# michaelnny/alpha_zero

Measured on AMD Instinct MI355X. Metric: self-play moves/sec (whole node), 9x9 Go @ 200 sims/move, higher is better.
Workload: dtype fp32-class evaluator (f16 hi+lo pairs, 3 MFMA products, fp32 accumulate) / f32-f64 tree

## Files before the change

alpha_zero_amd/csrc/azsp_hip.hip:

```cpp
#include <hip/hip_runtime.h>
#include <stdlib.h>

#include <type_traits>

#include "azsp_impl.h"
#include "az_conv64.h"
#include "az_conv19.h"
#include "az_conv_sp.h"
#include "az_conv_sp17.h"
#include "az_resblock_sp17.h"
#include "az_conv_sp2p.h"
#include "az_conv_spg.h"

static hipError_t g_last = hipSuccess;
#define AZ_HIP(x) ((g_last = (x)) == hipSuccess ? 0 : -1)

template <int N, int GAME, class Op>
__global__ void __launch_bounds__(256) k_game(const AzCfg c, const AzMem m, const Op op, const int g0, const int g1) {
    __shared__ typename Engine<WaveDev, N, GAME>::SC sc[4];
    const int wave = (int)(threadIdx.x >> 6);
    const int g = g0 + (int)blockIdx.x * 4 + wave;
    if (g >= g1) return;
    Engine<WaveDev, N, GAME> e(c, m, g, sc[wave]);
    op(e);
}

__global__ void __launch_bounds__(256) k_dihedral(const DihedralArgs a, long long total) {
    for (long long t = (long long)blockIdx.x * blockDim.x + threadIdx.x; t < total; t += (long long)gridDim.x * blockDim.x)
        az_dihedral_elem(a, t);
}

__global__ void __launch_bounds__(256) k_replay_gather(const ReplayGatherArgs a, long long total) {
    for (long long t = (long long)blockIdx.x * blockDim.x + threadIdx.x; t < total; t += (long long)gridDim.x * blockDim.x)
        az_replay_gather_elem(a, t);
}

__global__ void __launch_bounds__(256) k_bias_act(const BiasActArgs a) {
    for (long long i = (long long)blockIdx.x * blockDim.x + threadIdx.x; i < a.nvec; i += (long long)gridDim.x * blockDim.x)
        az_bias_act_vec(a, i);
}

__global__ void __launch_bounds__(1024) k_harvest_scan(const int* __restrict__ len, int* __restrict__ ofs, int* __restrict__ counts, int n2, int rot,
                                                        int cap, int max_games) {
    __shared__ int ss[1024], sg[1024], best[2];
    const int t = (int)threadIdx.x, per = (n2 + 1023) / 1024, lo = t * per < n2 ? t * per : n2, hi = lo + per < n2 ? lo + per : n2;
    int s = 0, g = 0;
    for (int i = lo; i < hi; ++i) {
        const int l = len[(i + rot) % n2];
        s += l;
        g += l > 0;
    }
    ss[t] = s;
    sg[t] = g;
    if (t < 2) best[t] = 0;
    __syncthreads();
    for (int d = 1; d < 1024; d <<= 1) {
        const int a = t >= d ? ss[t - d] : 0, b = t >= d ? sg[t - d] : 0;
        __syncthreads();
        ss[t] += a;
        sg[t] += b;
        __syncthreads();
    }
    int mine[2] = {0, 0};
    az_harvest_scan_range(len, ofs, n2, rot, cap, max_games, lo, hi, ss[t] - s, sg[t] - g, mine);
    if (mine[1] > 0) {
        atomicMax(&best[0], mine[0]);
        atomicMax(&best[1], mine[1]);
    }
    __syncthreads();
    if (t < 2) counts[t] = best[t];
}

namespace azb {
void* alloc(size_t n) {
    void* p = nullptr;
    if (AZ_HIP(hipMalloc(&p, n))) return nullptr;
    if (AZ_HIP(hipMemset(p, 0, n))) {
        hipFree(p);
        return nullptr;
    }
    return p;
}
void release(void* p) { (void)hipFree(p); }
int h2d(void* d, const void* s, size_t n, void* st) {
    if (AZ_HIP(hipMemcpyAsync(d, s, n, hipMemcpyHostToDevice, (hipStream_t)st))) return -1;
    return AZ_HIP(hipStreamSynchronize((hipStream_t)st));
}
int d2h(void* d, const void* s, size_t n, void* st) {
    if (AZ_HIP(hipMemcpyAsync(d, s, n, hipMemcpyDeviceToHost, (hipStream_t)st))) return -1;
    return AZ_HIP(hipStreamSynchronize((hipStream_t)st));
}
int zero(void* d, size_t n, void* st) { return AZ_HIP(hipMemsetAsync(d, 0, n, (hipStream_t)st)); }
int sync(void* st) { return AZ_HIP(hipStreamSynchronize((hipStream_t)st)); }
void* host_alloc(size_t n) {
    void* p = nullptr;
    return AZ_HIP(hipHostMalloc(&p, n, hipHostMallocDefault)) ? nullptr : p;
}
void host_release(void* p) { (void)hipHostFree(p); }
int set_device(int dev) {
    int n = 0;
    if (AZ_HIP(hipGetDeviceCount(&n)) || n < 1) return -1;
    return AZ_HIP(hipSetDevice(dev));
}
const char* backend_error() { return hipGetErrorString(g_last); }
template <class K, class... A> static int launch_k(K* kernel, unsigned grid, unsigned block, size_t lds, void* st, const A&... args) {
    hipLaunchKernelGGL(kernel, dim3(grid), dim3(block), lds, (hipStream_t)st, args...);
    return AZ_HIP(hipGetLastError());
}
template <class F> static int with_flag(bool flag, F&& f) { return flag ? f(std::true_type{}) : f(std::false_type{}); }
template <class F> static int with_flag(bool f0, bool f1, F&& f) {
    return with_flag(f0, [&](auto F0) { return with_flag(f1, [&](auto F1) { return f(decltype(F0){}, F1); }); });
}
static int cu_count() {
    static int n_cu = 0;
    if (n_cu == 0) {
        int dev = 0;
        hipDeviceProp_t prop;
        if (hipGetDevice(&dev) != hipSuccess || hipGetDeviceProperties(&prop, dev) != hipSuccess) return -1;
        n_cu = prop.multiProcessorCount > 0 ? prop.multiProcessorCount : 256;
    }
    return n_cu;
}
static int persistent_grid(long long units, int k = 1) {
    const int n_cu = cu_count();
    if (n_cu < 0) return -1;
    const long long slots = n_cu / k > 0 ? n_cu / k : 1;
    return k * (int)(units < slots ? units : slots);
}
template <int N, int GAME, class Op> int launch(const AzCfg& c, const AzMem& m, const Op& op, void* st, int g0, int g1) {
    return launch_k(k_game<N, GAME, Op>, (unsigned)((g1 - g0 + 3) / 4), 256, 0, st, c, m, op, g0, g1);
}
int launch_dihedral(const DihedralArgs& a, long long total, void* st) {
    long long blocks = (total + 255) / 256;
    if (blocks > 2048) blocks = 2048;
    return launch_k(k_dihedral, (unsigned)blocks, 256, 0, st, a, total);
}
int launch_replay_gather(const ReplayGatherArgs& a, long long total, void* st) {
    long long blocks = (total + 255) / 256;
    if (blocks > 256 * 16) blocks = 256 * 16;
    return launch_k(k_replay_gather, (unsigned)blocks, 256, 0, st, a, total);
}
int launch_harvest_scan(const int* len, int* ofs, int* counts, int n2, int rot, int cap, int max_games, void* st) {
    return launch_k(k_harvest_scan, 1, 1024, 0, st, len, ofs, counts, n2, rot, cap, max_games);
}
int launch_bias_act(const BiasActArgs& a, void* st) {
    long long blocks = (a.nvec + 255) / 256;
    if (blocks > 256 * 32) blocks = 256 * 32;
    return launch_k(k_bias_act, (unsigned)blocks, 256, 0, st, a);
}
int launch_conv3x3_tiled(const void* x, const void* w, const float* bias, const void* res, void* y, long long boards, int S, int C,
                         int relu, void* st, int f16) {
    if (f16 && (S != CV_S || C != CV_C)) return 1;
    const auto xb = (const unsigned char*)x, rb = (const unsigned char*)res;
    const auto wb = (const unsigned short*)w;
    const auto yb = (unsigned char*)y;
    if (C == C6_C && (S == 17 || S == 9)) {
        const long long ntiles = S == 17 ? boards : (boards + 2) / 3;
        const int grid = persistent_grid(ntiles);
        if (grid < 0) return -1;
        return with_flag(S == 17, res != nullptr, [&](auto G17, auto RES) {
            return launch_k(k_conv3x3_t64<C6Geo<G17 ? 17 : 9>, RES, 8>, grid, CW_THREADS, 0, st, xb, wb, bias, rb, yb, (int)ntiles, relu);
        });
    }
    if (S == C9_S && C == 256) {
        static const bool two_launch = getenv("AZSP_CONV19_TWO_LAUNCH") != nullptr;
        const int grid = persistent_grid(boards, two_launch ? 4 : 8);
        if (grid < 0) return -1;
        if (x == y || res == y) return 1;
        if (!two_launch) {
            return with_flag(res != nullptr, [&](auto RES) {
                return launch_k(k_conv3x3_op19q<RES>, grid, CW_THREADS, 0, st, xb, wb, bias, rb, yb, (int)boards, relu);
            });
        }
        const int rc = with_flag(res != nullptr, [&](auto RES) {
            return launch_k(k_conv3x3_hb19<RES, 16>, grid, CW_THREADS, 0, st, xb, wb, bias, rb, yb, (int)boards, 0, 1, 256, 0, 32, 0);
        });
        if (rc) return rc;
        return launch_k(k_conv3x3_hb19<true, 16>, grid, CW_THREADS, 0, st, xb, wb, bias, (const unsigned char*)yb, yb, (int)boards, relu, 0, 256, 128, 32, 16);
    }
    if (S != CV_S || C != CV_C) return 1;
    const long long ntiles = (boards + CV_TB - 1) / CV_TB;
    const int grid = persistent_grid(ntiles);
    if (grid < 0) return -1;
    return with_flag(res != nullptr, f16 != 0, [&](auto RES, auto F16) {
        return launch_k(k_conv3x3_tiled<RES, 16, F16>, grid, CW_THREADS, 0, st, xb, wb, bias, rb, yb, (int)ntiles, relu);
    });
}
int launch_resblock_tiled(const void* x, const void* w1, const float* b1, const void* w2, const float* b2, void* y, long long boards, int S, int C,
                          void* st) {
    if (C != C6_C || (S != 17 && S != 9)) return 1;
    const long long ntiles = S == 17 ? boards : (boards + 2) / 3;
    const int grid = persistent_grid(ntiles);
    if (grid < 0) return -1;
    return with_flag(S == 17, [&](auto G17) {
        return launch_k(k_resblock64<C6Geo<G17 ? 17 : 9>>, grid, CW_THREADS, 0, st, (const unsigned char*)x, (const unsigned short*)w1, b1,
                        (const unsigned short*)w2, b2, (unsigned char*)y, (int)ntiles);
    });
}
int launch_stem_tiled(const void* x, const void* w, const float* bias, void* y, long long boards, int S, int C, int pad, int relu, void* st, int f16) {
    if (f16 && (S != CV_S || C != CV_C || pad != 1)) return 1;
    const bool t64 = C == C6_C && ((S == 13 && pad == 3) || (S == 9 && pad == 1)), go19 = S == C9_S && C == 256 && pad == 1;
    if (!t64 && !go19 && (S != CV_S || C != CV_C || pad != 1)) return 1;
    const long long ntiles = t64 ? (S == 13 ? boards : (boards + 2) / 3) : go19 ? boards : (boards + CV_TB - 1) / CV_TB;
    const int grid = persistent_grid(ntiles, go19 ? 4 : 1);
    if (grid < 0) return -1;
    const auto xb = (const unsigned char*)x, nores = (const unsigned char*)nullptr;
    const auto wb = (const unsigned short*)w;
    const auto yb = (unsigned char*)y;
    if (t64)
        return with_flag(S == 13, [&](auto G17) {
            return launch_k(k_conv3x3_t64<C6Geo<G17 ? 17 : 9>, false, 4>, grid, CW_THREADS, 0, st, xb, wb, bias, nores, yb, (int)ntiles, relu);
        });
    if (go19) return launch_k(k_conv3x3_hb19<false, 4>, grid, CW_THREADS, 0, st, xb, wb, bias, nores, yb, (int)boards, relu, 1, 32, 0, 4, 0);
    return with_flag(f16 != 0, [&](auto F16) {
        return launch_k(k_conv3x3_tiled<false, 4, F16>, grid, CW_THREADS, 0, st, xb, wb, bias, nores, yb, (int)ntiles, relu);
    });
}
int launch_head_tiled(const void* x, const float* w, const float* bias, void* pol, void* val, long long boards, int S, int C, int npol, int nval,
                      int pol_stride, int val_stride, void* st, int f16) {
    if (C % 8 || C > 1024 || npol + nval != 3) return 1;
    const long long npos = boards * S * S;
    return with_flag(f16 != 0, [&](auto F16) {
        return launch_k(k_head_tiled<3, F16>, (unsigned)((npos + 255) / 256), 256, 0, st, (const unsigned char*)x, w, bias, (unsigned short*)pol,
                        (unsigned short*)val, npos, npol, C, S * S, cv_tile_boards(S) * S * S, pol_stride, val_stride);
    });
}
template <int T1, int T2, bool F16> static int launch_fc_heads_t(const FcHeadsArgs& a, void* st) {
    return launch_k(k_fc_heads<T1, T2, F16>, (unsigned)((a.boards + 127) / 128), 256, 0, st, (const unsigned short*)a.pol, (const unsigned short*)a.val,
                    (const unsigned short*)a.wp, a.bp, a.ks1, (const unsigned short*)a.w1, a.b1, a.ks2, a.w2, a.b2, a.priors, a.values, a.boards, a.A);
}
int launch_fc_heads(const FcHeadsArgs& a, void* st) {
    const int nt1 = (a.A + 31) / 32, nt2 = (a.F + 31) / 32;
    if (a.f16) return nt1 == 3 && nt2 == 4 ? launch_fc_heads_t<3, 4, true>(a, st) : 1;
    if (nt1 == 3 && nt2 == 2) return launch_fc_heads_t<3, 2, false>(a, st);
    if (nt1 == 3 && nt2 == 4) return launch_fc_heads_t<3, 4, false>(a, st);
    if (nt1 == 6 && nt2 == 2) return launch_fc_heads_t<6, 2, false>(a, st);
    if (nt1 == 6 && nt2 == 4) return launch_fc_heads_t<6, 4, false>(a, st);
    if (nt1 == 12 && nt2 == 8) return launch_fc_heads_t<12, 8, false>(a, st);
    return 1;
}
int launch_tile_layout(const void* src, void* dst, long long boards, int S, int C, int to_tiled, void* st) {
    if (C % 8 || S < 1) return 1;
    const int nch = C / 8, tile_rows = cv_tile_boards(S) * S * S;
    const long long nchunks = boards * S * S * nch;
    return launch_k(k_tile_layout, (unsigned)((nchunks + 255) / 256), 256, 0, st, (const unsigned char*)src, (unsigned char*)dst, nchunks, to_tiled, nch,
                    tile_rows);
}
int launch_split_layout(const void* src, void* dst, long long boards, int S, int C, int to_split, void* st, unsigned* range) {
    if (C % 8 || S < 1) return 1;
    const long long nchunks = boards * S * S * (C / 8);
    return launch_k(k_split_layout, (unsigned)((nchunks + 255) / 256), 256, 0, st, (const unsigned char*)src, (unsigned char*)dst, nchunks, to_split, C / 8,
                    S * S, range);
}
template <bool RES, int NCH, int NCG, bool XLO0 = false>
static int launch_sp(const void* x, const void* w, const float* bias, const void* res, void* y, long long boards, int relu, void* st, unsigned* range) {
    const int grid = persistent_grid(boards, NCG);
    if (grid < 0) return -1;
    return launch_k(k_conv3x3_sp<RES, NCH, NCG, XLO0>, grid, CW_THREADS, 0, st, (const unsigned char*)x, (const _Float16*)w, bias, (const unsigned char*)res,
                    (unsigned char*)y, (int)boards, relu, range);
}
template <bool RES, int NCH, bool XLO0 = false>
static int launch_sp17(const void* x, const void* w, const float* bias, const void* res, void* y, long long boards, int relu, void* st, unsigned* range) {
    const int grid = persistent_grid(boards);
    if (grid < 0) return -1;
    return launch_k(k_conv3x3_sp17<RES, NCH, XLO0>, grid, CW_THREADS, 0, st, (const unsigned char*)x, (const _Float16*)w, bias, (const unsigned char*)res,
                    (unsigned char*)y, (int)boards, relu, range);
}
static long long spg_wave_items(long long boards, int S, int C, int NT, int NJ) {
    const long long nct = ((long long)S * S + 15) / 16;
    return boards * ((nct + NJ - 1) / NJ) * (C / (16 * NT));
}
static unsigned spg_wave_grid(long long boards, int S, int C, int NT, int NJ) {
    const long long grid = (spg_wave_items(boards, S, C, NT, NJ) + 3) / 4;
    return grid > 0x7fffffffLL ? 0u : (unsigned)grid;
}
template <bool RES, int KSUB, int NT, int NJ, int HALVES>
static int launch_spg_t(const void* x, const void* w, const float* bias, const void* res, void* y, long long boards, int S, int C, int relu, void* st,
                        unsigned* range) {
    const unsigned grid = spg_wave_grid(boards, S, C, NT, NJ);
    if (!grid) return 1;
    return launch_k(k_conv3x3_spg<RES, KSUB, NT, NJ, HALVES>, grid, 256, 0, st, (const unsigned char*)x, (const _Float16*)w, bias,
                    (const unsigned char*)(RES ? res : nullptr), (unsigned char*)y, (int)boards, S, C, relu, range);
}
template <bool RES, int KSUB, int NT>
static int launch_spgw_t(const void* x, const void* w, const float* bias, const void* res, void* y, long long boards, int S, int C, int relu, void* st,
                         unsigned* range) {
    const long long nct = ((long long)S * S + 15) / 16, grid = (boards * ((nct + 2) / 3) * (C / (64 * NT)) + 7) / 8 * 8;
    if (grid > 0x7fffffffLL || C % (64 * NT)) return 1;
    return launch_k(k_conv3x3_spgw<RES, KSUB, NT>, (unsigned)grid, 256, 0, st, (const unsigned char*)x, (const _Float16*)w, bias,
                    (const unsigned char*)(RES ? res : nullptr), (unsigned char*)y, (int)boards, S, C, relu, range);
}
template <int KSUB, int HALVES>
static int launch_spg_k(const void* x, const void* w, const float* bias, const void* res, void* y, long long boards, int S, int C, int relu, void* st,
                        unsigned* range, bool latency) {
    constexpr int NT = KSUB == 2 ? 1 : 2;
    return with_flag(res != nullptr, [&](auto RES) {
        return latency || HALVES == 2 ? launch_spg_t<RES, KSUB, 1, 2, HALVES>(x, w, bias, res, y, boards, S, C, relu, st, range)
                                      : launch_spgw_t<RES, KSUB, NT>(x, w, bias, res, y, boards, S, C, relu, st, range);
    });
}
static int launch_spg(const void* x, const void* w, const float* bias, const void* res, void* y, long long boards, int S, int C, int relu, void* st,
                      unsigned* range, bool latency, int halves) {
    if (S < 3 || S > 64 || boards < 1 || boards > 0x7fffffffLL) return 1;
    if (C == 64) return launch_spg_k<2, 1>(x, w, bias, res, y, boards, S, C, relu, st, range, latency);
    if (C == 128)
        return halves == 2 ? launch_spg_k<4, 2>(x, w, bias, res, y, boards, S, C, relu, st, range, latency)
                           : launch_spg_k<4, 1>(x, w, bias, res, y, boards, S, C, relu, st, range, latency);
    if (C == 256) return launch_spg_k<8, 1>(x, w, bias, res, y, boards, S, C, relu, st, range, latency);
    return 1;
}
static constexpr long long SPG_DEFAULT_WAVES = 1024;
static long long& spg_max_waves() {
    static long long n = [] {
        const char* e = getenv("AZSP_SPG_MAX_WAVES");
        const long long v = e ? atoll(e) : SPG_DEFAULT_WAVES;
        return v < 0 ? 0LL : v;
    }();
    return n;
}
static bool small_batch(long long boards, int S, int C) { return spg_wave_items(boards, S, C, 1, 2) <= spg_max_waves(); }
long long small_batch_waves(long long n) {
    const long long old = spg_max_waves();
    if (n >= 0) spg_max_waves() = n;
    return old;
}
int launch_conv3x3_split(const void* x, const void* w, const float* bias, const void* res, void* y, long long boards, int S, int C, int relu,
                         void* st, unsigned* range) {
    const bool sp17 = S == Sp17Geo::S && C == 64, sp9 = S == SpGeo9::S && (C == 128 || C == 64), small = small_batch(boards, S, C);
    if (!(sp17 || sp9) || small) return launch_spg(x, w, bias, res, y, boards, S, C, relu, st, range, small, sp9 && C == 128 ? 2 : 1);
    if (sp17)
        return with_flag(res != nullptr, [&](auto RES) { return launch_sp17<RES, 8>(x, w, bias, res, y, boards, relu, st, range); });
    if (C == 64) return with_flag(res != nullptr, [&](auto RES) { return launch_sp<RES, 8, 1>(x, w, bias, res, y, boards, relu, st, range); });
    const long long pairs = boards / 2;
    const int pgrid = persistent_grid(pairs, 2);
    if (pgrid < 0) return -1;
    const size_t off = (size_t)(2 * pairs) * 2 * 128 * SpGeo9::P2 * 2;
    const auto xb = (const unsigned char*)x, rb = (const unsigned char*)res;
    const auto yb = (unsigned char*)y;
    const int rc = with_flag(res != nullptr, [&](auto RES) {
        return pairs > 0 ? launch_k(k_conv3x3_sp2p<RES>, pgrid, CW_THREADS, 0, st, xb, (const _Float16*)w, bias, rb, yb, (int)pairs, relu, range) : 0;
    });
    if (rc || !(boards & 1)) return rc;
    return launch_spg(xb + off, w, bias, res ? rb + off : nullptr, yb + off, 1, S, C, relu, st, range, true, 2);
}
enum Scratch {
    SCRATCH_SPG_BLOCK,
    SCRATCH_COUNT
};
static constexpr long long SPG_SCRATCH_BOARDS = 256;
static void* device_scratch(Scratch which, size_t bytes) {
    static void* buf[SCRATCH_COUNT][16] = {};
    int dev = 0;
    if (hipGetDevice(&dev) != hipSuccess || dev < 0 || dev >= 16) return nullptr;
    if (!buf[which][dev] && AZ_HIP(hipMalloc(&buf[which][dev], bytes))) return nullptr;
    return buf[which][dev];
}
static int launch_resblock_spg(const unsigned char* x, const void* w1, const float* b1, const void* w2, const float* b2, unsigned char* y, long long boards,
                               int S, int C, void* st, unsigned* range) {
    void* mid = device_scratch(SCRATCH_SPG_BLOCK, (size_t)SPG_SCRATCH_BOARDS * 2 * 8 * Sb17::S * Sb17::S * 16);
    if (!mid) return -1;
    const int rc = launch_spg(x, w1, b1, nullptr, mid, boards, S, C, 1, st, range, true, 1);
    if (rc) return rc;
    return launch_spg(mid, w2, b2, x, y, boards, S, C, 1, st, range, true, 1);
}
int launch_resblock_split(const void* x, const void* w1, const float* b1, const void* w2, const float* b2, void* y, long long boards, int S, int C,
                          void* st, unsigned* range) {
    if (C != 64 || (S != Sb17::S && S != Sb9::S)) return 1;
    const long long pairs = boards / 2;
    const int grid = persistent_grid(S == Sb9::S ? pairs : boards);
    if (grid < 0) return -1;
    const auto xb = (const unsigned char*)x;
    const auto yb = (unsigned char*)y;
    if (small_batch(boards, S, C) && boards <= SPG_SCRATCH_BOARDS) return launch_resblock_spg(xb, w1, b1, w2, b2, yb, boards, S, C, st, range);
    if (S == Sb17::S) return launch_k(k_resblock_sp<Sb17, 6>, grid, CW_THREADS, 0, st, xb, (const _Float16*)w1, b1, (const _Float16*)w2, b2, yb, (int)boards, range);
    if (pairs > 0 && launch_k(k_resblock_sp<Sb9, 6>, grid, CW_THREADS, 0, st, xb, (const _Float16*)w1, b1, (const _Float16*)w2, b2, yb, (int)pairs, range)) return -1;
    if (!(boards & 1)) return 0;
    const size_t off = (size_t)(boards - 1) * Sb9::GTILEB;
    return launch_resblock_spg(xb + off, w1, b1, w2, b2, yb + off, 1, S, C, st, range);
}
int launch_split_features(const float* src, void* dst, long long boards, int S, int cin, void* st, unsigned* range) {
    if (cin < 1 || cin > 32 || S < 1) return 1;
    const long long nitems = boards * 4 * S * S;
    return launch_k(k_split_features, (unsigned)((nitems + 255) / 256), 256, 0, st, src, (unsigned char*)dst, nitems, cin, S * S, range);
}
template <bool XLO0>
static int launch_stem_spg(const void* x, const void* w, const float* bias, void* y, long long boards, int n, int C, int pad, int relu, void* st,
                           unsigned* range) {
    constexpr int NT = 1, NJ = 2;
    const int off = pad - 1, S = n + 2 * off;
    if ((pad != 1 && pad != 3) || n < 1 || S < 3 || S > 64 || (C != 64 && C != 128 && C != 256) || boards < 1 || boards > 0x7fffffffLL) return 1;
    const unsigned grid = spg_wave_grid(boards, S, C, NT, NJ);
    if (!grid) return 1;
    return launch_k(k_stem_spg<XLO0, NT, NJ>, grid, 256, 0, st, (const unsigned char*)x, (const _Float16*)w, bias, (unsigned char*)y, (int)boards, n, off,
                    C, relu, range);
}
static constexpr bool STEM_SPG_DEFAULT_SMALL = false;
int launch_stem_split(const void* x, const void* w, const float* bias, void* y, long long boards, int S, int C, int pad, int relu, void* st,
                      int x_lo_zero, unsigned* range) {
    const bool sp17 = S == 13 && C == 64 && pad == 3;
    const bool sp9 = S == SpGeo9::S && (C == 128 || C == 64) && pad == 1;
    const bool small = (pad == 1 || pad == 3) && small_batch(boards, S + 2 * (pad - 1), C) && (STEM_SPG_DEFAULT_SMALL || spg_max_waves() > SPG_DEFAULT_WAVES);
    return with_flag(x_lo_zero != 0, [&](auto XLO0) {
        if (!(sp17 || sp9) || small) return launch_stem_spg<XLO0>(x, w, bias, y, boards, S, C, pad, relu, st, range);
        if (sp17) return launch_sp17<false, 4, XLO0>(x, w, bias, nullptr, y, boards, relu, st, range);
        return C == 128 ? launch_sp<false, 4, 2, XLO0>(x, w, bias, nullptr, y, boards, relu, st, range)
                        : launch_sp<false, 4, 1, XLO0>(x, w, bias, nullptr, y, boards, relu, st, range);
    });
}
int split_range_read(const unsigned* rec, unsigned out[2], int reset, void* st) {
    void* p = (void*)rec;
    if (!p && AZ_HIP(hipGetSymbolAddress(&p, HIP_SYMBOL(g_sp_range)))) return -1;
    if (AZ_HIP(hipMemcpyAsync(out, p, 2 * sizeof(unsigned), hipMemcpyDeviceToHost, (hipStream_t)st))) return -1;
    if (reset && AZ_HIP(hipMemsetAsync(p, 0, 2 * sizeof(unsigned), (hipStream_t)st))) return -1;
    return AZ_HIP(hipStreamSynchronize((hipStream_t)st));
}
template <int BPB> static int launch_head_split_bpb(const HeadSplitArgs& a, void* st) {
    const int P2 = a.S * a.S;
    const size_t lds = (size_t)(BPB * (3 * ((P2 + 3) & ~3) + a.A + a.F)) * sizeof(float);
    if (lds > 64 * 1024) return 1;
    return launch_k(k_head_split<BPB>, (unsigned)((a.boards + BPB - 1) / BPB), 256, lds, st, (const unsigned char*)a.x, a.hw, a.hb, a.wp_t, a.bp, a.w1_t, a.b1, a.w2,
                    a.b2, a.priors, a.values, a.boards, a.C, P2, a.A, a.F, a.npol);
}
int launch_head_split(const HeadSplitArgs& a, void* st) {
    if (a.C % 8 || a.npol < 1 || a.npol > 2) return 1;
    return launch_head_split_bpb<4>(a, st);
}
}
```

Baseline: 7347.

## Add dedicated persistent pipelined stem conv kernel for 9x9 boards with 128 channels

Adds a specialized persistent stem kernel for 9x9, 128-channel, 32-input-channel boards. It keeps weights resident in registers, streams boards through an LDS ring with asynchronous DMA, and interleaves each board's epilogue stores with the next board's MFMA products. Corner cells are gathered into a side buffer and computed in batches of 16 boards. The goal is to hide load and store latency that the generic sp stem path exposes, at the cost of a lot of hand-scheduled code, high register pressure and one block per CU.

```diff
diff --git a/alpha_zero_amd/csrc/az_stem_sp9.h b/alpha_zero_amd/csrc/az_stem_sp9.h
--- /dev/null
+++ b/alpha_zero_amd/csrc/az_stem_sp9.h
@@ -0,0 +1,273 @@
+#pragma once
+#include <type_traits>
+
+#include "az_conv_sp.h"
+
+#if defined(__HIPCC__)
+#ifndef SP9_RING
+#define SP9_RING 4
+#endif
+#ifndef SP9_CELL16
+#define SP9_CELL16 true
+#endif
+
+template <bool XLO0> struct Sp9K {
+    typedef SpGeo9 G;
+    static constexpr int NR = SP9_RING;
+    static constexpr int NCH = 4, C = 128, CIN = 32, KS = 9, R = 3, NT = G::NCT;
+    static constexpr int NPROD = XLO0 ? 2 : 3, NQ = 2 * NPROD;
+    static constexpr int NPL = XLO0 ? 1 : 2;
+    static constexpr int LBLK = G::CELLS * 16, LPLANE = NCH * LBLK, LBUF = NPL * LPLANE;
+    static constexpr int GBLK = G::P2 * 16, XPLANE = NCH * GBLK, XTILE = 2 * XPLANE;
+    static constexpr int YPLANE = (C / 8) * GBLK, YTILE = 2 * YPLANE;
+    static constexpr int NP = (G::CELLS + 63) / 64, SPW = NPL * NCH / 4, NPW = NP * SPW;
+    static constexpr int NST = SP9_CELL16 ? 2 : 4;
+    static constexpr int ARITH = 2 * 2 * sp_epi_pair(false), CT_OPS = ARITH + NST;
+    static constexpr int S0 = 6;
+    static constexpr int BAR_T = KS - (R - 1);
+    typedef SpSpread<CT_OPS, S0, KS * NQ - 4 - S0> SpreadMid;
+    typedef SpSpread<CT_OPS, S0, BAR_T * NQ - S0> SpreadLast;
+    static constexpr int SIDE_BOARD = 8 * NCH * 16 + 16, SIDE0 = NR * LBUF + 16, LDS_BYTES = SIDE0 + 16 * SIDE_BOARD;
+    static constexpr int VM_PIECES = (NR - 2) * NPW, VM_COUNT = VM_PIECES + NT * NST * (NR - 2) + (NT - 1) * NST, VM_STEADY = VM_COUNT < 62 ? VM_COUNT : 62;
+    static_assert(NR >= 2 && NR <= 8, "ring depth");
+    static_assert((NT * KS) % R == 0, "a board's k-steps keep the fragment ring's phase");
+    static_assert(LPLANE + (2 * G::PITCH + 2) * 16 < 65536, "fragment addresses are a base + a 16-bit immediate");
+    static_assert(LDS_BYTES <= 160 * 1024, "LDS budget");
+};
+
+template <bool XLO0> __global__ void __launch_bounds__(CW_THREADS, 1)
+k_stem_sp9(const unsigned char* __restrict__ x, const _Float16* __restrict__ w, const float* __restrict__ bias, unsigned char* __restrict__ y,
+           int ntiles, int relu, unsigned* range) {
+    typedef SpGeo9 G;
+    typedef Sp9K<XLO0> K;
+    constexpr int NR = K::NR, NCH = K::NCH, C = K::C, CIN = K::CIN, KS = K::KS, R = K::R, NT = K::NT, NPROD = K::NPROD, NQ = K::NQ, NPL = K::NPL;
+    constexpr int LBLK = K::LBLK, LPLANE = K::LPLANE, LBUF = K::LBUF, GBLK = K::GBLK, XTILE = K::XTILE, YPLANE = K::YPLANE, YTILE = K::YTILE;
+    constexpr int NP = K::NP, SPW = K::SPW, NPW = K::NPW, NST = K::NST, ARITH = K::ARITH, CT_OPS = K::CT_OPS;
+    constexpr int SIDE_BOARD = K::SIDE_BOARD, SIDE0 = K::SIDE0;
+    constexpr int NF = 2 * KS * 2;
+    __shared__ __attribute__((aligned(1024))) unsigned char lds[K::LDS_BYTES];
+    const int tid = threadIdx.x, lane = tid & 63, l15 = lane & 15, kg = lane >> 4;
+    const int wave = __builtin_amdgcn_readfirstlane(tid >> 6);
+    const unsigned lds0 = (unsigned)(size_t)(__attribute__((address_space(3))) unsigned char*)lds;
+    const int slot = (int)blockIdx.x, nslot = (int)gridDim.x;
+    for (int i = tid; i < K::LDS_BYTES / 16; i += CW_THREADS) *(cv_u32x4*)(lds + i * 16) = (cv_u32x4){0u, 0u, 0u, 0u};
+    CV_BARRIER();
+    if (slot >= ntiles) return;
+
+    sp_f16x8 wf[NF];
+#pragma unroll
+    for (int f = 0; f < NF; ++f) {
+        const int r = f & 1, pt = f >> 1;
+        wf[f] = *(const sp_f16x8*)(w + ((size_t)(pt * C + wave * 32 + 8 * (l15 >> 2) + (l15 & 3) + 4 * r)) * CIN + kg * 8);
+    }
+    c6_f32x4 bv[2];
+#pragma unroll
+    for (int r = 0; r < 2; ++r)
+#pragma unroll
+        for (int e = 0; e < 4; ++e) bv[r][e] = bias[wave * 32 + 8 * kg + 4 * r + e];
+    const float lo_relu = relu ? 0.0f : -__builtin_inff();
+    const float lo_clamp = relu ? 0.0f : -SP_F16_MAX;
+
+    unsigned dsrc[NP];
+    unsigned long long dmask[NP];
+    sp_dma_plan(dsrc, dmask, lane, [](int cell) { return cell < G::CELLS ? G::pos_of_cell(cell) * 16 : -1; });
+    auto dma_board = [&](long long tile, int rs) __attribute__((always_inline)) {
+        const bool live = tile < ntiles;
+        const unsigned char* src = x + (size_t)(live ? tile : slot) * XTILE;
+        const unsigned dst = lds0 + (unsigned)(rs * LBUF);
+#pragma unroll
+        for (int i = 0; i < NPW; ++i) sp_dma_piece(src, dst, SPW * wave + i / NP, i % NP, GBLK, LBLK, live ? dmask[i % NP] : 0ull, dsrc[i % NP]);
+    };
+    unsigned lmap[NT], omap[NT];
+#pragma unroll
+    for (int j = 0; j < NT; ++j) {
+        const int pos = sp_map9.pos[j * 16 + l15];
+        lmap[j] = (unsigned)((G::PITCH * (pos / G::S) + pos % G::S) * 16 + kg * LBLK);
+        omap[j] = (unsigned)(pos * 16 + kg * GBLK);
+    }
+    auto out_off = [&](int j) __attribute__((always_inline)) {
+        unsigned v = omap[j];
+        asm volatile("" : "+v"(v));
+        return v;
+    };
+    sp_f16x8 bb[R][2];
+    auto load_frag = [&](unsigned img, int j, int t, int rs, int pl) __attribute__((always_inline)) {
+        bb[rs][pl] = *(const sp_f16x8*)(lds + img + lmap[j] + sp_frag_off(t, 1, G::PITCH, LBLK) + pl * LPLANE);
+    };
+
+#pragma unroll
+    for (int b = 0; b < NR; ++b) dma_board(slot + (long long)b * nslot, b);
+    asm volatile("s_waitcnt vmcnt(%0)" ::"n"((NR - 1) * NPW) : "memory");
+    CV_BARRIER();
+#pragma unroll
+    for (int s = 0; s < R - 1; ++s)
+#pragma unroll
+        for (int pl = 0; pl < NPL; ++pl) load_frag(0u, 0, s, s, pl);
+#pragma unroll
+    for (int f = 0; f < NF; ++f) asm volatile("" : : "a"(wf[f]));
+    asm volatile("" : : "v"(bv[0]), "v"(bv[1]), "v"(lmap[0]), "v"(lmap[NT - 1]), "v"(dsrc[0]), "v"(dsrc[NP - 1]));
+
+    c6_f32x4 accm[2][2] = {}, accc[2][2] = {};
+    const cv_u32x2 nores[2] = {};
+    SpEpi ep[2];
+    auto epi_op = [&](int set, int mj, const SpOut& out, int o, bool store_ok) __attribute__((always_inline)) {
+        if (o < ARITH) {
+            const int r = o / (ARITH / 2);
+            ep[r].op<false>(o % (ARITH / 2), accm[set][r], accc[set][r], nores, lo_clamp);
+        } else if (store_ok) {
+            const int st = o - ARITH;
+            const unsigned off = out_off(mj);
+            if constexpr (SP9_CELL16) {
+                if (st == 0) *(cv_u32x4*)(out.hi + off) = (cv_u32x4){ep[0].hpk[0], ep[0].hpk[1], ep[1].hpk[0], ep[1].hpk[1]};
+                else *(__attribute__((address_space(1))) cv_u32x4*)(out.lo + off) = (cv_u32x4){ep[0].lpk[0], ep[0].lpk[1], ep[1].lpk[0], ep[1].lpk[1]};
+            } else {
+                const int r = st >> 1;
+                if ((st & 1) == 0) *(cv_u32x2*)(out.hi + off + 8 * r) = (cv_u32x2){ep[r].hpk[0], ep[r].hpk[1]};
+                else *(__attribute__((address_space(1))) cv_u32x2*)(out.lo + off + 8 * r) = (cv_u32x2){ep[r].lpk[0], ep[r].lpk[1]};
+            }
+        }
+    };
+
+    const bool copier = tid < 8 * NCH && (!XLO0 || !(tid & 1));
+    int csrc, cdst;
+    {
+        const int c = tid < 8 * NCH ? tid : 0, pl = c & 1, tp = (c >> 1) & 3, g4 = c >> 3;
+        csrc = (XLO0 ? 0 : pl * LPLANE) + g4 * LBLK + (G::CELL0 + G::PITCH * (G::S - 2 + (tp >> 1)) + (tp & 1)) * 16;
+        cdst = SIDE0 + c * 16;
+    }
+    cv_u32x4 ctmp = (cv_u32x4){0u, 0u, 0u, 0u};
+
+    int it = 0;
+    SpOut yprev = {y, (sp_gptr)(unsigned long long)y};
+    for (int tile = slot; tile < ntiles; tile += nslot, ++it) {
+        const int rslot = it % NR;
+        const unsigned Xs = (unsigned)(rslot * LBUF), Xn = (unsigned)((rslot + 1 == NR ? 0 : rslot + 1) * LBUF);
+        const bool has_next = tile + nslot < ntiles;
+        const size_t yo = (size_t)tile * YTILE + (size_t)(wave * 4) * GBLK;
+        const SpOut ybase = sp_out_base(y + yo, YPLANE);
+        const bool have_prev = it > 0;
+        auto board = [&](auto PC) __attribute__((always_inline)) {
+            constexpr int PAR = decltype(PC)::value;
+            cp_for_each([&](auto JC) __attribute__((always_inline)) {
+                constexpr int j = decltype(JC)::value, set = (PAR + j) & 1, pset = set ^ 1;
+                constexpr int pmj = j == 0 ? NT - 1 : j - 1;
+                typedef typename std::conditional<j == NT - 1, typename K::SpreadLast, typename K::SpreadMid>::type SP;
+                const SpOut pout = j == 0 ? yprev : ybase;
+                const bool pstore = j > 0 || have_prev;
+                cp_for_each([&](auto TC) __attribute__((always_inline)) {
+                    constexpr int t = decltype(TC)::value;
+                    constexpr int g = j * KS + t;
+                    if constexpr (j == NT - 1 && t == K::BAR_T) {
+                        if (it >= NR - 1) asm volatile("s_waitcnt vmcnt(%0)" ::"n"(K::VM_STEADY) : "memory");
+                        else asm volatile("s_waitcnt vmcnt(%0)" ::"n"(K::VM_PIECES) : "memory");
+                        CV_BARRIER();
+                        dma_board(tile + (long long)NR * nslot, rslot);
+                    }
+                    constexpr int lg = g + R - 1, lrs = lg % R;
+                    constexpr bool lsame = lg < NT * KS;
+                    constexpr int lj = lsame ? lg / KS : 0, lt = lsame ? lg % KS : lg - NT * KS;
+                    const unsigned limg = lsame ? Xs : Xn;
+                    cp_for_each([&](auto QC) __attribute__((always_inline)) {
+                        constexpr int q = decltype(QC)::value, r = q & 1, prod = XLO0 ? (q < 2 ? 0 : 2) : q >> 1;
+                        if constexpr (q < NPL) load_frag(limg, lj, lt, lrs, q);
+                        constexpr int fa = ((prod == 2 ? KS : 0) + t) * 2 + r, pl = prod == 1 ? 1 : 0;
+                        if constexpr (prod == 0) {
+                            if constexpr (t == 0) sp_mfma_ac(accm[set][r], wf[fa], bb[g % R][pl], bv[r]);
+                            else sp_mfma_a(accm[set][r], wf[fa], bb[g % R][pl]);
+                        } else if constexpr (t == 0 && prod == (XLO0 ? 2 : 1)) {
+                            sp_mfma_a0(accc[set][r], wf[fa], bb[g % R][pl]);
+                        } else {
+                            sp_mfma_a(accc[set][r], wf[fa], bb[g % R][pl]);
+                        }
+                        constexpr int sl = t * NQ + q;
+                        cp_for_each([&](auto KC) __attribute__((always_inline)) {
+                            constexpr int o = SP::cum(sl - 1) + decltype(KC)::value;
+                            if constexpr (o < SP::cum(sl)) epi_op(pset, pmj, pout, o, pstore);
+                        }, typename CpMakeSeq<SP::MAXPER>::type{});
+                        __builtin_amdgcn_sched_barrier(0);
+                    }, typename CpMakeSeq<NQ>::type{});
+                    if constexpr (j == 0 && t == 2) {
+                        if (copier) ctmp = *(const cv_u32x4*)(lds + Xs + csrc);
+                    }
+                    if constexpr (j == 0 && t == 5) {
+                        if (copier) *(cv_u32x4*)(lds + cdst + (it & 15) * SIDE_BOARD) = ctmp;
+                    }
+                    __builtin_amdgcn_sched_barrier(0);
+                }, typename CpMakeSeq<KS>::type{});
+            }, typename CpMakeSeq<NT>::type{});
+        };
+        if (it & 1) board(CpInt<1>{});
+        else board(CpInt<0>{});
+        yprev = ybase;
+        if ((it & 15) == 15 || !has_next) {
+            const int n_ok = (it & 15) + 1, it0 = it - (it & 15);
+            c6_f32x4 cm[2], cc[2];
+            const unsigned char* sb = lds + SIDE0 + l15 * SIDE_BOARD + kg * (8 * 16);
+            const int nb = l15 < n_ok ? l15 : 0;
+            const size_t co = (size_t)(slot + (size_t)(it0 + nb) * nslot) * YTILE + (size_t)(wave * 4 + kg) * GBLK + G::CORNER * 16;
+            sp_f16x8 fb[2][2];
+            fb[0][0] = *(const sp_f16x8*)(sb);
+            if constexpr (!XLO0) fb[0][1] = *(const sp_f16x8*)(sb + 16);
+            cp_for_each([&](auto TC) __attribute__((always_inline)) {
+                constexpr int u = decltype(TC)::value;
+                constexpr int tp = ((u >> 1) * 3 + 1 + (u & 1));
+                if constexpr (u + 1 < 4) {
+                    fb[(u + 1) & 1][0] = *(const sp_f16x8*)(sb + ((u + 1) * 2 + 0) * 16);
+                    if constexpr (!XLO0) fb[(u + 1) & 1][1] = *(const sp_f16x8*)(sb + ((u + 1) * 2 + 1) * 16);
+                }
+                const sp_f16x8& bh = fb[u & 1][0];
+#pragma unroll
+                for (int r = 0; r < 2; ++r) {
+                    if constexpr (u == 0) sp_mfma_ac(cm[r], wf[tp * 2 + r], bh, bv[r]);
+                    else sp_mfma_a(cm[r], wf[tp * 2 + r], bh);
+                }
+                if constexpr (!XLO0) {
+                    const sp_f16x8& bl = fb[u & 1][1];
+#pragma unroll
+                    for (int r = 0; r < 2; ++r) {
+                        if constexpr (u == 0) sp_mfma_a0(cc[r], wf[tp * 2 + r], bl);
+                        else sp_mfma_a(cc[r], wf[tp * 2 + r], bl);
+                    }
+                }
+#pragma unroll
+                for (int r = 0; r < 2; ++r) {
+                    if constexpr (XLO0 && u == 0) sp_mfma_a0(cc[r], wf[(KS + tp) * 2 + r], bh);
+                    else sp_mfma_a(cc[r], wf[(KS + tp) * 2 + r], bh);
+                }
+                __builtin_amdgcn_sched_barrier(0);
+            }, typename CpMakeSeq<4>::type{});
+            asm volatile("s_nop 15\n\ts_nop 15" : "+v"(cm[0]), "+v"(cm[1]), "+v"(cc[0]), "+v"(cc[1]));
+            unsigned hw[4], lw[4];
+#pragma unroll
+            for (int r = 0; r < 2; ++r) {
+                float v[4];
+                _Float16 h[4], l[4];
+#pragma unroll
+                for (int e = 0; e < 4; ++e) {
+                    v[e] = fmaxf(fmaf(cc[r][e], SP_INV_SCALE, cm[r][e]), lo_relu);
+                    if (l15 < n_ok) ep[0].mx = fmaxf(ep[0].mx, fabsf(v[e]));
+                    sp_split(v[e], h[e], l[e]);
+                }
+                hw[2 * r] = sp_pack(h[0], h[1]), hw[2 * r + 1] = sp_pack(h[2], h[3]);
+                lw[2 * r] = sp_pack(l[0], l[1]), lw[2 * r + 1] = sp_pack(l[2], l[3]);
+            }
+            if (l15 < n_ok) {
+                *(cv_u32x4*)(y + co) = (cv_u32x4){hw[0], hw[1], hw[2], hw[3]};
+                *(cv_u32x4*)(y + co + YPLANE) = (cv_u32x4){lw[0], lw[1], lw[2], lw[3]};
+            }
+            CV_BARRIER();
+        }
+    }
+    asm volatile("s_nop 15\n\ts_nop 15" : "+v"(accm[0][0]), "+v"(accm[0][1]), "+v"(accc[0][0]), "+v"(accc[0][1]), "+v"(accm[1][0]), "+v"(accm[1][1]),
+                 "+v"(accc[1][0]), "+v"(accc[1][1]));
+    if ((it - 1) & 1) {
+#pragma unroll
+        for (int o = 0; o < CT_OPS; ++o) epi_op(1, NT - 1, yprev, o, true);
+    } else {
+#pragma unroll
+        for (int o = 0; o < CT_OPS; ++o) epi_op(0, NT - 1, yprev, o, true);
+    }
+    sp_range_report(fmaxf(ep[0].mx, ep[1].mx), range);
+}
+
+#endif
diff --git a/alpha_zero_amd/csrc/azsp_hip.hip b/alpha_zero_amd/csrc/azsp_hip.hip
--- a/alpha_zero_amd/csrc/azsp_hip.hip
+++ b/alpha_zero_amd/csrc/azsp_hip.hip
@@ -11,6 +11,7 @@
 #include "az_resblock_sp17.h"
 #include "az_conv_sp2p.h"
 #include "az_conv_spg.h"
+#include "az_stem_sp9.h"
 
 static hipError_t g_last = hipSuccess;
 #define AZ_HIP(x) ((g_last = (x)) == hipSuccess ? 0 : -1)
@@ -384,6 +385,12 @@
     return launch_k(k_split_features, (unsigned)((nitems + 255) / 256), 256, 0, st, src, (unsigned char*)dst, nitems, cin, S * S, range);
 }
 template <bool XLO0>
+static int launch_stem_sp9(const void* x, const void* w, const float* bias, void* y, long long boards, int relu, void* st, unsigned* range) {
+    const int grid = persistent_grid(boards);
+    if (grid < 0) return -1;
+    return launch_k(k_stem_sp9<XLO0>, grid, CW_THREADS, 0, st, (const unsigned char*)x, (const _Float16*)w, bias, (unsigned char*)y, (int)boards, relu, range);
+}
+template <bool XLO0>
 static int launch_stem_spg(const void* x, const void* w, const float* bias, void* y, long long boards, int n, int C, int pad, int relu, void* st,
                            unsigned* range) {
     constexpr int NT = 1, NJ = 2;
@@ -403,7 +410,7 @@
     return with_flag(x_lo_zero != 0, [&](auto XLO0) {
         if (!(sp17 || sp9) || small) return launch_stem_spg<XLO0>(x, w, bias, y, boards, S, C, pad, relu, st, range);
         if (sp17) return launch_sp17<false, 4, XLO0>(x, w, bias, nullptr, y, boards, relu, st, range);
-        return C == 128 ? launch_sp<false, 4, 2, XLO0>(x, w, bias, nullptr, y, boards, relu, st, range)
+        return C == 128 ? launch_stem_sp9<XLO0>(x, w, bias, y, boards, relu, st, range)
                         : launch_sp<false, 4, 1, XLO0>(x, w, bias, nullptr, y, boards, relu, st, range);
     });
 }
```

Result: no change. 7394 (median of 6 runs) (+0.6%).
